# yongjianxu/ompi-release

Hardware: AMD Instinct MI355X
Metric: MPI_Allreduce busbw GB/s (1 GiB fp32, np=8) + op/hip reduce HBM GB/s (higher is better)
Workload: dtype f32; 1 GPU; op/hip 3-buff MPI_SUM MPI_FLOAT, 1 GiB per operand (BASELINE configs[1]); count=268435456, bytes_per_operand=1073741824

## Files before the change

### include/coll_mi355x.h

```cpp
#ifndef MI355X_COLL_MI355X_H
#define MI355X_COLL_MI355X_H

#include "ompi_abi.h"

#ifdef __cplusplus
extern "C" {
#endif

extern mca_coll_base_component_t mca_coll_mi355x_component;

int mca_coll_mi355x_allreduce(void *sbuf, void *rbuf, int count, struct ompi_datatype_t *dtype,
                              struct ompi_op_t *op, struct ompi_communicator_t *comm,
                              mca_coll_base_module_t *module);
int mca_coll_mi355x_reduce(void *sbuf, void *rbuf, int count, struct ompi_datatype_t *dtype, struct ompi_op_t *op,
                           int root, struct ompi_communicator_t *comm, mca_coll_base_module_t *module);
int mca_coll_mi355x_iallreduce(void *sbuf, void *rbuf, int count, struct ompi_datatype_t *dtype, struct ompi_op_t *op,
                               struct ompi_communicator_t *comm, ompi_request_t **request,
                               mca_coll_base_module_t *module);
int mca_coll_mi355x_iscan(void *sbuf, void *rbuf, int count, struct ompi_datatype_t *dtype, struct ompi_op_t *op,
                          struct ompi_communicator_t *comm, ompi_request_t **request, mca_coll_base_module_t *module);
int mca_coll_mi355x_iexscan(void *sbuf, void *rbuf, int count, struct ompi_datatype_t *dtype, struct ompi_op_t *op,
                            struct ompi_communicator_t *comm, ompi_request_t **request, mca_coll_base_module_t *module);
int mca_coll_mi355x_ireduce(void *sbuf, void *rbuf, int count, struct ompi_datatype_t *dtype, struct ompi_op_t *op,
                            int root, struct ompi_communicator_t *comm, ompi_request_t **request,
// ... 72 lines not shown
                                   ompi_request_t **request);
int mca_coll_mi355x_pml_irecv_init(void *buf, size_t count, struct ompi_datatype_t *dt, int src, int tag,
                                   struct ompi_communicator_t *comm, ompi_request_t **request);
int mca_coll_mi355x_pml_start(size_t count, ompi_request_t **requests);

extern int mca_coll_mi355x_priority;
extern int mca_coll_mi355x_allreduce_algorithm;
extern int mca_coll_mi355x_pml_hook;
extern int mca_coll_mi355x_mixed_buffers;
extern int mca_coll_mi355x_rcache_max_maps;
extern unsigned long long mca_coll_mi355x_rcache_size_limit;
extern int mca_coll_mi355x_pipe_min_ranks;
extern int mca_coll_mi355x_pipe_chunk_kib;
extern int mca_coll_mi355x_pipe_wg_per_cu;
extern int mca_coll_mi355x_pipe_wt;
extern unsigned long long mca_coll_mi355x_one_phase_max;
extern unsigned long long mca_coll_mi355x_svc_max;
extern unsigned long long mca_coll_mi355x_svc_pull_max;
extern unsigned long long mca_coll_mi355x_svc_copy_max;
extern int mca_coll_mi355x_svc_idle_us;
extern int mca_coll_mi355x_svc_shrink_us;
extern int mca_coll_mi355x_selftest;
extern int mca_coll_mi355x_nb_order;
extern unsigned long long mca_coll_mi355x_scan_part_min;
struct mi355x_comm *mca_coll_mi355x_engine_of(struct ompi_communicator_t *comm);

extern unsigned long mca_coll_mi355x_staged_calls;
int mca_coll_mi355x_reducible_type(const struct ompi_datatype_t *dt);

#ifdef __cplusplus
// ... 4 lines not shown
```

### include/mi355x_rt.h

```cpp
#ifndef MI355X_RT_H
#define MI355X_RT_H

#include <stddef.h>
#include <stdint.h>

#include "mi355x_types.h"

#ifdef __cplusplus
extern "C" {
#endif

const char *mi355x_last_error(void);
int mi355x_version(void);
int mi355x_device_count(int *count);
int mi355x_set_device(int dev);
int mi355x_get_device(int *dev);
int mi355x_stream_create(void **stream);
int mi355x_stream_destroy(void *stream);
int mi355x_stream_sync(void *stream);
int mi355x_device_sync(void);
int mi355x_malloc(void **p, size_t bytes);
int mi355x_free(void *p);
int mi355x_host_alloc(void **p, size_t bytes);
int mi355x_host_free(void *p);
// ... 23 lines not shown
int mi355x_op_set_threads(int threads);


typedef struct mi355x_comm mi355x_comm_t;

int mi355x_comm_create(const char *key, int rank, int size, int device, mi355x_comm_t **comm);
int mi355x_comm_create_loopback(int size, int device, mi355x_comm_t **comms);
int mi355x_comm_destroy(mi355x_comm_t *comm);
int mi355x_comm_rank(const mi355x_comm_t *comm);
int mi355x_comm_size(const mi355x_comm_t *comm);
int mi355x_comm_barrier(mi355x_comm_t *comm);
int mi355x_comm_vote(mi355x_comm_t *comm, int device, int *engine);
int mi355x_comm_last_algorithm(const mi355x_comm_t *comm);
int mi355x_debug_pipe_token(mi355x_comm_t *comm, int acquire);
int mi355x_debug_token(uint64_t dev_uid, const char *name, int op);

enum mi355x_knob {
    MI355X_KNOB_ALLREDUCE_ALG = 1,
    MI355X_KNOB_REDUCE_ALG = 2,
    MI355X_KNOB_REDUCE_SCATTER_ALG = 3,
    MI355X_KNOB_BLOCKS_PER_CU = 4,
    MI355X_KNOB_TIMEOUT_S = 5,
    MI355X_KNOB_PUSH = 6,
    MI355X_KNOB_IPC_MAX_BYTES = 7,
    MI355X_KNOB_STAGE_BYTES = 8,
    MI355X_KNOB_REDUCE_CHAIN_FANOUT = 10,
    MI355X_KNOB_LL_MAX_BYTES = 9,
    MI355X_KNOB_TIME_PHASES = 11,
    MI355X_KNOB_COPY_BLOCK_KIB = 12,
    MI355X_KNOB_PIPE = 13,
// ... 16 lines not shown
    MI355X_KNOB_FLOWS_FAILED = 30,
    MI355X_KNOB_CREATE_US = 31,
    MI355X_KNOB_SELFTEST_US = 32,
    MI355X_KNOB_SVC_OWNER = 33,
    MI355X_KNOB_SVC_CLAIMS = 34,
    MI355X_KNOB_SVC_IDLE_US = 35,
    MI355X_KNOB_SVC_SHRINK_US = 36,
    MI355X_KNOB_SVC_REGROWS = 37,
    MI355X_KNOB_DEV_SETUP = 38,
    MI355X_KNOB_SETUP_US = 39,
    MI355X_KNOB_SELFTEST = 40,
    MI355X_KNOB_PIPE_CALLS = 41,
    MI355X_KNOB_EXPORT_MISMATCHES = 42,
    MI355X_KNOB_SELFTEST_REUSED = 43,
    MI355X_KNOB_NB_ORDER = 44,
    MI355X_KNOB_SCAN_PART_MIN_BYTES = 45
};
enum mi355x_flow {
    MI355X_FLOW_SVC_LL = 1,
    MI355X_FLOW_SVC_PULL = 2,
    MI355X_FLOW_SVC_COPY = 4,
    MI355X_FLOW_SVC_RS = 8,
    MI355X_FLOW_PIPE = 16
};
int mi355x_comm_set(mi355x_comm_t *comm, int knob, long value);
int mi355x_comm_get(const mi355x_comm_t *comm, int knob, long *value);
int mi355x_comm_phase_ms(const mi355x_comm_t *comm, float *phase1_ms, float *phase2_ms);

enum mi355x_coll_id {
    MI355X_COLL_ALLGATHER = 0, MI355X_COLL_ALLREDUCE = 2, MI355X_COLL_BCAST = 7, MI355X_COLL_REDUCE = 11,
// ... 127 lines not shown
```

### ompi-release_amd/__init__.py

```python
from __future__ import annotations

import ctypes
import os
import pathlib

PKG_DIR = pathlib.Path(__file__).resolve().parent
LIB_DIR = pathlib.Path(os.environ["MI355X_LIB_DIR"]) if os.environ.get("MI355X_LIB_DIR") else PKG_DIR / "lib"
REPO_DIR = PKG_DIR.parent

TYPES = [
    "INT8", "UINT8", "INT16", "UINT16", "INT32", "UINT32", "INT64", "UINT64",
    "F_INTEGER", "F_INTEGER1", "F_INTEGER2", "F_INTEGER4", "F_INTEGER8", "F_INTEGER16",
    "FLOAT", "DOUBLE", "F_REAL", "F_REAL2", "F_REAL4", "F_REAL8", "F_REAL16",
    "F_DOUBLE_PRECISION", "LONG_DOUBLE", "F_LOGICAL", "BOOL",
    "C_FLOAT_COMPLEX", "C_DOUBLE_COMPLEX", "C_LONG_DOUBLE_COMPLEX", "BYTE",
    "F_2REAL", "F_2DOUBLE_PRECISION", "F_2INTEGER",
    "FLOAT_INT", "DOUBLE_INT", "LONG_INT", "2INT", "SHORT_INT", "LONG_DOUBLE_INT", "WCHAR",
]
T = {name: i for i, name in enumerate(TYPES)}
OPS = ["NULL", "MAX", "MIN", "SUM", "PROD", "LAND", "BAND", "LOR", "BOR", "LXOR", "BXOR",
       "MAXLOC", "MINLOC", "REPLACE", "NO_OP"]
OP = {name: i for i, name in enumerate(OPS)}

MI355X_SUCCESS = 0
# ... 73 lines not shown
        "mi355x_op_reduce_3buff": (i, [i, i, vp, vp, vp, sz, vp]),
        "mi355x_op_tune": (i, [i, i, i]),
        "mi355x_op_get_tune": (i, [c.POINTER(i), c.POINTER(i), c.POINTER(i)]),
        "mi355x_op_set_mode": (i, [i]),
        "mi355x_op_get_mode": (i, []),
        "mi355x_op_set_threads": (i, [i]),
        "mi355x_comm_create": (i, [c.c_char_p, i, i, i, c.POINTER(vp)]),
        "mi355x_comm_create_loopback": (i, [i, i, c.POINTER(vp)]),
        "mi355x_comm_destroy": (i, [vp]),
        "mi355x_comm_rank": (i, [vp]),
        "mi355x_comm_size": (i, [vp]),
        "mi355x_comm_barrier": (i, [vp]),
        "mi355x_comm_last_algorithm": (i, [vp]),
        "mi355x_debug_pipe_token": (i, [vp, i]),
        "mi355x_debug_token": (i, [c.c_uint64, c.c_char_p, i]),
        "mi355x_comm_set": (i, [vp, i, c.c_long]),
        "mi355x_comm_phase_ms": (i, [vp, c.POINTER(c.c_float), c.POINTER(c.c_float)]),
        "mi355x_comm_get": (i, [vp, i, c.POINTER(c.c_long)]),
        "mi355x_allreduce": (i, [vp, vp, vp, sz, i, i, vp]),
        "mi355x_reduce_scatter_block": (i, [vp, vp, vp, sz, i, i, vp]),
        "mi355x_reduce": (i, [vp, vp, vp, sz, i, i, i, vp]),
        "mi355x_iallreduce": (i, [vp, vp, vp, sz, i, i, vp, c.POINTER(vp)]),
        "mi355x_ireduce": (i, [vp, vp, vp, sz, i, i, i, vp, c.POINTER(vp)]),
        "mi355x_ireduce_scatter_block": (i, [vp, vp, vp, sz, i, i, vp, c.POINTER(vp)]),
        "mi355x_ireduce_scatter": (i, [vp, vp, vp, c.POINTER(i), i, i, vp, c.POINTER(vp)]),
        "mi355x_iallgather": (i, [vp, vp, vp, sz, vp, c.POINTER(vp)]),
        "mi355x_ibcast": (i, [vp, vp, sz, i, vp, c.POINTER(vp)]),
        "mi355x_request_test": (i, [vp, c.POINTER(i)]),
        "mi355x_request_wait": (i, [vp]),
        "mi355x_request_free": (i, [vp]),
# ... 105 lines not shown


def get_tune() -> tuple[int, int, int]:
    a, b, c = ctypes.c_int(), ctypes.c_int(), ctypes.c_int()
    check(rt().mi355x_op_get_tune(ctypes.byref(a), ctypes.byref(b), ctypes.byref(c)))
    return a.value, b.value, c.value


def scan_part_plan(count: int, n: int, q: int, r: int) -> tuple[int, int, int | None]:
    a, b, c_ = ctypes.c_size_t(), ctypes.c_size_t(), ctypes.c_size_t()
    check(rt().mi355x_scan_part_plan(count, n, q, r, ctypes.byref(a), ctypes.byref(b), ctypes.byref(c_)),
          "mi355x_scan_part_plan")
    return a.value, b.value, None if r == q else c_.value


KNOB = {"ALLREDUCE_ALG": 1, "REDUCE_ALG": 2, "REDUCE_SCATTER_ALG": 3, "BLOCKS_PER_CU": 4, "TIMEOUT_S": 5,
        "PUSH": 6, "IPC_MAX_BYTES": 7, "STAGE_BYTES": 8,
        "LL_MAX_BYTES": 9, "REDUCE_CHAIN_FANOUT": 10, "TIME_PHASES": 11,
        "COPY_BLOCK_KIB": 12, "PIPE": 13, "PIPE_WG_PER_CU": 14, "PIPE_CHUNK_KIB": 15, "PIPE_WT": 16,
        "ONE_PHASE_MAX_BYTES": 17, "PIPE_REFUSED": 18, "SVC_MAX_BYTES": 19, "SVC_CALLS": 20,
        "SVC_LAUNCHES": 21, "SVC_RESIDENT": 22, "SVC_PULL_MAX_BYTES": 23,
        "SVC_PULL_COPY_MAX_BYTES": 24, "RCACHE_MAX_MAPS": 25, "RCACHE_SIZE_LIMIT": 26, "PEER_MAPS": 27,
        "RCACHE_EVICTIONS": 28, "FLOWS": 29, "FLOWS_FAILED": 30, "CREATE_US": 31, "SELFTEST_US": 32,
        "SVC_OWNER": 33, "SVC_CLAIMS": 34, "SVC_IDLE_US": 35,
        "SVC_SHRINK_US": 36, "SVC_REGROWS": 37, "DEV_SETUP": 38, "SETUP_US": 39, "SELFTEST": 40,
        "PIPE_CALLS": 41, "EXPORT_MISMATCHES": 42, "SELFTEST_REUSED": 43, "NB_ORDER": 44,
        "SCAN_PART_MIN_BYTES": 45}
NBC_ALG = {"BINOMIAL": 101, "RING": 102, "CHAIN": 103}
FLOW = {"SVC_LL": 1, "SVC_PULL": 2, "SVC_COPY": 4, "SVC_RS": 8, "PIPE": 16}
COLL = {"ALLGATHER": 0, "ALLREDUCE": 2, "BCAST": 7, "REDUCE": 11, "REDUCESCATTER": 12}
AR_ALG = {"DECISION": 0, "LINEAR": 1, "NONOVERLAPPING": 2, "RECURSIVE_DOUBLING": 3, "RING": 4,
          "RING_SEGMENTED": 5}


class Comm:

    def __init__(self, handle: int):
        self.h = ctypes.c_void_p(handle)

    @classmethod
    def create(cls, key: str, rank: int, size: int, device: int) -> "Comm":
        h = ctypes.c_void_p()
# ... 374 lines not shown
```

### ompi-release_amd/csrc/mca/coll/mi355x/coll_mi355x_component.c

```c
#include <stdio.h>
#include <stdlib.h>
#include <string.h>
#include <time.h>
#include <unistd.h>

#include "../../../../../include/coll_mi355x.h"
#include "../../../../../include/mi355x_rt.h"

int mca_coll_mi355x_priority = 90;
int mca_coll_mi355x_allreduce_algorithm = 0;
int mca_coll_mi355x_pml_hook = 1;

typedef struct mca_coll_mi355x_module_t {
    mca_coll_base_module_t super;
    mi355x_comm_t *engine;
    mca_coll_base_module_allreduce_fn_t prev_allreduce;
    mca_coll_base_module_t *prev_allreduce_module;
    mca_coll_base_module_reduce_scatter_fn_t prev_reduce_scatter;
    mca_coll_base_module_t *prev_reduce_scatter_module;
    mca_coll_base_module_reduce_scatter_block_fn_t prev_reduce_scatter_block;
    mca_coll_base_module_t *prev_reduce_scatter_block_module;
    mca_coll_base_module_allgather_fn_t prev_allgather;
    mca_coll_base_module_t *prev_allgather_module;
    mca_coll_base_module_bcast_fn_t prev_bcast;
// ... 244 lines not shown
    default:
        fprintf(stderr, "[coll/mi355x] %s\n", mi355x_last_error());
        return OMPI_ERROR;
    }
}

#define MOD(m) ((mca_coll_mi355x_module_t *)(m))

int mca_coll_mi355x_mixed_buffers = 1;
int mca_coll_mi355x_rcache_max_maps = 0;
unsigned long long mca_coll_mi355x_rcache_size_limit = 0;
int mca_coll_mi355x_pipe_min_ranks = 4;
int mca_coll_mi355x_pipe_chunk_kib = 0;
int mca_coll_mi355x_pipe_wg_per_cu = 2;
int mca_coll_mi355x_pipe_wt = 1;
unsigned long long mca_coll_mi355x_one_phase_max = 1ull << 20;
unsigned long long mca_coll_mi355x_svc_max = 32ull << 10;
unsigned long long mca_coll_mi355x_svc_pull_max = 128ull << 10;
unsigned long long mca_coll_mi355x_svc_copy_max = 1ull << 20;
int mca_coll_mi355x_svc_idle_us = 1000;
int mca_coll_mi355x_svc_shrink_us = 100;
int mca_coll_mi355x_selftest = 1;
int mca_coll_mi355x_nb_order = 0;
unsigned long long mca_coll_mi355x_scan_part_min = 0;
int mca_coll_mi355x_timeout_s = 0;

static int route(mca_coll_mi355x_module_t *m, int dev)
{
    if (!m->mixed) return dev;
    int engine = dev;
// ... 1740 lines not shown
    return OMPI_ERR_BAD_PARAM;
}

static int apply_engine_params(mca_coll_mi355x_module_t *m, struct ompi_communicator_t *comm)
{
    const int n = mi355x_comm_size_of(comm);
    int rc = OMPI_SUCCESS;
#define KNOB(K, V, NAME) if (rc == OMPI_SUCCESS) rc = set_knob(m, MI355X_KNOB_##K, (long)(V), NAME)
    KNOB(SELFTEST, mca_coll_mi355x_selftest != 0, "selftest");
    KNOB(NB_ORDER, mca_coll_mi355x_nb_order != 0, "nb_order");
    KNOB(SCAN_PART_MIN_BYTES, mca_coll_mi355x_scan_part_min, "scan_part_min_bytes");
    KNOB(PIPE, mca_coll_mi355x_pipe_min_ranks > 0 && n >= mca_coll_mi355x_pipe_min_ranks, "pipe_min_ranks");
    KNOB(PIPE_CHUNK_KIB, mca_coll_mi355x_pipe_chunk_kib, "pipe_chunk_kib");
    KNOB(PIPE_WG_PER_CU, mca_coll_mi355x_pipe_wg_per_cu, "pipe_wg_per_cu");
    KNOB(PIPE_WT, mca_coll_mi355x_pipe_wt != 0, "pipe_wt");
    KNOB(ONE_PHASE_MAX_BYTES, mca_coll_mi355x_one_phase_max, "one_phase_max");
    KNOB(SVC_MAX_BYTES, mca_coll_mi355x_svc_max, "svc_max");
    KNOB(SVC_PULL_MAX_BYTES, mca_coll_mi355x_svc_pull_max, "svc_pull_max");
    KNOB(SVC_PULL_COPY_MAX_BYTES, mca_coll_mi355x_svc_copy_max, "svc_copy_max");
    KNOB(SVC_IDLE_US, mca_coll_mi355x_svc_idle_us, "svc_idle_us");
    KNOB(SVC_SHRINK_US, mca_coll_mi355x_svc_shrink_us, "svc_shrink_us");
    if (mca_coll_mi355x_timeout_s > 0) KNOB(TIMEOUT_S, mca_coll_mi355x_timeout_s, "timeout_s");
#undef KNOB
    return rc;
}

struct mi355x_comm *mca_coll_mi355x_engine_of(struct ompi_communicator_t *comm)
{
    if (!comm || comm->c_coll.coll_allreduce != mca_coll_mi355x_allreduce || !comm->c_coll.coll_allreduce_module)
        return NULL;
// ... 94 lines not shown
                 "allgather / bcast (every rank votes its buffer kind; 0: every rank must use the same kind)",
                 OPAL_INFO_LVL_5, &mca_coll_mi355x_mixed_buffers);
    register_int("rcache_max_maps", "Most mappings of peers' device allocations kept open per communicator; the least "
                 "recently used beyond it are closed (0 = unlimited)", OPAL_INFO_LVL_9, &mca_coll_mi355x_rcache_max_maps);
    register_ull("rcache_size_limit", "The same bound in bytes of mapped peer allocations, as mpool_rgpusm_rcache_size_limit "
                 "(0 = unlimited)", OPAL_INFO_LVL_9, &mca_coll_mi355x_rcache_size_limit);
    register_int("pipe_min_ranks", "Communicators of at least this many ranks run large allreduces through the "
                 "pipelined copy||reduce flow (one persistent launch, per-chunk flags); 0 = never", OPAL_INFO_LVL_5,
                 &mca_coll_mi355x_pipe_min_ranks);
    register_int("pipe_chunk_kib", "Chunk size of the pipelined allreduce in KiB (0 = about 512 chunks per ring block)",
                 OPAL_INFO_LVL_6, &mca_coll_mi355x_pipe_chunk_kib);
    register_int("pipe_wg_per_cu", "Workgroups per CU of the pipelined allreduce (1..8)", OPAL_INFO_LVL_6,
                 &mca_coll_mi355x_pipe_wg_per_cu);
    register_int("pipe_wt", "Pipelined allreduce: 1 = fold results stored write-through with system-scope ready flags, "
                 "0 = stored and released by the producer's fence", OPAL_INFO_LVL_9, &mca_coll_mi355x_pipe_wt);
    register_ull("one_phase_max", "Per-rank message bytes up to which an allreduce runs the one-launch ring-ordered flow "
                 "instead of the two-phase one", OPAL_INFO_LVL_6, &mca_coll_mi355x_one_phase_max);
    register_ull("svc_max", "Per-rank message bytes up to which small allreduce / reduce / allgather / bcast / "
                 "reduce_scatter_block calls go to the resident LL service in its LL form (svc_max, svc_pull_max and "
                 "svc_copy_max all 0: no service)", OPAL_INFO_LVL_5,
                 &mca_coll_mi355x_svc_max);
    register_ull("svc_pull_max", "Per-rank bytes up to which the service serves allreduce in its pull form (above "
                 "svc_max)", OPAL_INFO_LVL_6, &mca_coll_mi355x_svc_pull_max);
    register_ull("svc_copy_max", "Per-rank bytes up to which the service copies allgather / bcast (above svc_max)",
                 OPAL_INFO_LVL_6, &mca_coll_mi355x_svc_copy_max);
    register_int("svc_idle_us", "Idle time after which the resident service's kernel leaves the GPU, microseconds "
                 "(100 .. 60000000)", OPAL_INFO_LVL_6, &mca_coll_mi355x_svc_idle_us);
    register_int("svc_shrink_us", "Idle time after which the resident service shrinks to one workgroup, microseconds "
                 "(0 = never)", OPAL_INFO_LVL_6, &mca_coll_mi355x_svc_shrink_us);
    register_int("selftest", "Run the cross-device flows' self-tests at a communicator's first device-buffer collective "
// ... 85 lines not shown
```

### ompi-release_amd/csrc/rt/coll_comm.cpp

```cpp

#include <fcntl.h>
#include <immintrin.h>
#include <poll.h>
#include <sched.h>
#include <signal.h>
#include <sys/mman.h>
#include <sys/socket.h>
#include <sys/stat.h>
#include <sys/un.h>
#include <unistd.h>

#include <algorithm>
#include <array>
#include <atomic>
#include <cerrno>
#include <chrono>
#include <condition_variable>
#include <cstddef>
#include <deque>
#include <functional>
#include <cstdio>
#include <cstdlib>
#include <cstring>
#include <map>
// ... 349 lines not shown
    case MI355X_KNOB_REDUCE_SCATTER_ALG: *value = c->knob_rs; break;
    case MI355X_KNOB_BLOCKS_PER_CU: *value = c->tune.blocks_per_cu; break;
    case MI355X_KNOB_TIMEOUT_S: *value = (long)c->timeout_s; break;
    case MI355X_KNOB_PUSH: *value = c->tune.push; break;
    case MI355X_KNOB_IPC_MAX_BYTES: *value = (long)c->ipc_max; break;
    case MI355X_KNOB_STAGE_BYTES: *value = (long)c->stage_bytes; break;
    case MI355X_KNOB_PIPE_REFUSED: *value = (long)c->pipe_refused; break;
    case MI355X_KNOB_LL_MAX_BYTES: *value = (long)c->ll_max; break;
    case MI355X_KNOB_REDUCE_CHAIN_FANOUT: *value = c->chain_fanout; break;
    case MI355X_KNOB_TIME_PHASES: *value = c->time_phases ? 1 : 0; break;
    case MI355X_KNOB_COPY_BLOCK_KIB: *value = c->tune.copy_block_kib; break;
    case MI355X_KNOB_PIPE: *value = c->pipe_on ? 1 : 0; break;
    case MI355X_KNOB_PIPE_WG_PER_CU: *value = c->tune.pipe_wg_per_cu; break;
    case MI355X_KNOB_PIPE_CHUNK_KIB: *value = c->tune.pipe_chunk_kib; break;
    case MI355X_KNOB_PIPE_WT: *value = c->tune.pipe_wt; break;
    case MI355X_KNOB_ONE_PHASE_MAX_BYTES: *value = (long)c->one_phase_max; break;
    case MI355X_KNOB_SVC_MAX_BYTES: *value = svc_limit_visible(c) ? (long)c->svc_max : 0; break;
    case MI355X_KNOB_SVC_CALLS: *value = (long)c->svc_calls; break;
    case MI355X_KNOB_SVC_LAUNCHES: *value = (long)c->svc_launches; break;
    case MI355X_KNOB_SVC_RESIDENT: *value = c->svcq && svc_resident(c->svcq) ? 1 : 0; break;
    case MI355X_KNOB_SVC_PULL_MAX_BYTES: *value = svc_limit_visible(c) ? (long)c->svc_pull_max : 0; break;
    case MI355X_KNOB_SVC_PULL_COPY_MAX_BYTES: *value = svc_limit_visible(c) ? (long)c->svc_copy_max : 0; break;
    case MI355X_KNOB_FLOWS: *value = (long)c->flows; break;
    case MI355X_KNOB_FLOWS_FAILED: *value = (long)c->flows_failed; break;
    case MI355X_KNOB_CREATE_US: *value = (long)c->create_us; break;
    case MI355X_KNOB_SELFTEST_US: *value = (long)c->selftest_us; break;
    case MI355X_KNOB_SELFTEST_REUSED: *value = (long)c->selftest_reused; break;
    case MI355X_KNOB_DEV_SETUP: *value = c->dev_ready ? 1 : 0; break;
    case MI355X_KNOB_SELFTEST: *value = c->selftest ? 1 : 0; break;
    case MI355X_KNOB_PIPE_CALLS: *value = (long)c->pipe_calls; break;
// ... 64 lines not shown
        break;
    case MI355X_KNOB_COPY_BLOCK_KIB:
        if (value < 4 || value > 256) return set_error(MI355X_ERR_ARG, "copy_block_kib out of range");
        c->tune.copy_block_kib = (int)value;
        break;
    case MI355X_KNOB_PIPE: c->pipe_on = value != 0 && (c->flows & MI355X_FLOW_PIPE); break;
    case MI355X_KNOB_PIPE_WG_PER_CU:
        if (value < 1 || value > 8) return set_error(MI355X_ERR_ARG, "pipe_wg_per_cu out of range");
        c->tune.pipe_wg_per_cu = (int)value;
        break;
    case MI355X_KNOB_PIPE_CHUNK_KIB:
        if (value < 0 || value > (1l << 20)) return set_error(MI355X_ERR_ARG, "pipe_chunk_kib out of range");
        c->tune.pipe_chunk_kib = (int)value;
        break;
    case MI355X_KNOB_PIPE_WT: c->tune.pipe_wt = value != 0; break;
    case MI355X_KNOB_ONE_PHASE_MAX_BYTES:
        if (value < 0 || value > (1l << 30)) return set_error(MI355X_ERR_ARG, "one_phase_max_bytes out of range");
        c->one_phase_max = (size_t)value;
        break;
    case MI355X_KNOB_TIME_PHASES:
        c->time_phases = value != 0;
        if (c->time_phases && !c->tev[0]) {
            DeviceGuard dg(c->device);
            for (hipEvent_t &e : c->tev) MI_HIP(hipEventCreate(&e));
        }
        break;
    case MI355X_KNOB_LL_MAX_BYTES:
        if (value < 0 || value > (64l << 20)) return set_error(MI355X_ERR_ARG, "ll_max_bytes out of range");
        c->ll_max = c->ll_ok ? (size_t)value : 0;
        break;
// ... 121 lines not shown
```

### ompi-release_amd/csrc/rt/coll_internal.hpp

```cpp
#pragma once

#include <hip/hip_runtime.h>

#include <cstddef>
#include <cstdint>

namespace mi355x {

constexpr int kMaxRanks = 64;
constexpr int kFoldChunk = 8;
constexpr int kTreeMax = 16;
constexpr int kTreeSteps = 64;

struct FoldArgs {
    const void *src[kMaxRanks];
    void *dst[kMaxRanks];
    int order[kMaxRanks];
    uint64_t role_mask;
    int nr;
    int nd;
    size_t n;
    size_t head, nvec;
    int three;
};
// ... 120 lines not shown
    const void *src[kMaxRanks];
    const char *peer_rbuf[kMaxRanks];
    char *dst;
    uint64_t *peer_flag[kMaxRanks];
    const uint64_t *my_flag;
    uint64_t *queue;
    uint32_t *err;
    uint64_t qbase, seq, timeout_ticks, kmax, chunk, count;
    uint64_t boff[kMaxRanks], blen[kMaxRanks];
    uint64_t role_mask;
    uint64_t co_pull;
    int order[kMaxRanks];
    int n, me, co_fold;
    int wt;
    uint32_t nchunks;
    uint64_t *dbg;
};
int launch_pipe_slot(int op, int type, const PipeArgs &a, unsigned grid, hipStream_t s);
int pipe_blocks_per_cu(int op, int type, size_t count);

struct CollTune {
    int blocks_per_cu = 1024;
    int copy_block_kib = 4;
    int push = 0;
    int pipe_wg_per_cu = 2;
    int pipe_chunk_kib = 0;
    int pipe_wt = 1;
};
CollTune &coll_tune();
CollTune &coll_tune_default();
CollTune *coll_tune_use(CollTune *t);

int launch_fold_slot(int op, int type, const FoldArgs &a, hipStream_t s);
int launch_scan_slot(int op, int type, const ScanArgs &a, hipStream_t s);
int launch_ring_all_slot(int op, int type, const RingAllArgs &a, hipStream_t s);
int launch_tree_slot(int op, int type, const TreeArgs &a, hipStream_t s);
int launch_copy(CopyArgs a, hipStream_t s);
int launch_multicopy(MultiCopyArgs a, hipStream_t s);

}
```

### ompi-release_amd/csrc/rt/coll_pipe.hip

```cpp
#include "coll_internal.hpp"
#include "op_functors.hpp"
#include "rt_internal.hpp"
#include "slot_list.hpp"

namespace mi355x {

typedef unsigned int u32x4p __attribute__((ext_vector_type(4)));

template <typename T> struct alignas(16) PVec {
    T e[16 / sizeof(T)];
};

template <bool NT> __device__ __forceinline__ u32x4p pload(const void *p)
{
    if constexpr (NT) return __builtin_nontemporal_load(reinterpret_cast<const u32x4p *>(p));
    return *reinterpret_cast<const u32x4p *>(p);
}
template <bool NT> __device__ __forceinline__ void pstore(void *p, const u32x4p &v)
{
    if constexpr (NT) __builtin_nontemporal_store(v, reinterpret_cast<u32x4p *>(p));
    else *reinterpret_cast<u32x4p *>(p) = v;
}

constexpr int kSysCoherent = 1 | 16;
// ... 142 lines not shown
}

template <class F, bool NT> __global__ __launch_bounds__(256) void k_pipe_allreduce(PipeArgs a)
{
    using T = typename F::T;
    constexpr size_t esz = sizeof(T);
    __shared__ uint64_t item_s;
    __shared__ uint32_t give_up_s;
    const uint64_t total = (uint64_t)a.nchunks * (uint64_t)a.n;
    for (;;) {
        if (threadIdx.x == 0) item_s = __hip_atomic_fetch_add(a.queue, 1ull, __ATOMIC_RELAXED, __HIP_MEMORY_SCOPE_AGENT) - a.qbase;
        __syncthreads();
        const uint64_t it = uniform64(item_s);
        if (threadIdx.x == 0) dbg_store(a, 0, it);
        if (it >= total) break;
        if (it < a.nchunks) {
            const uint64_t k = it;
            const size_t blen = a.blen[a.me], lo = k * a.chunk, hi = lo + a.chunk < blen ? lo + a.chunk : blen;
            const bool wt = a.wt && a.co_fold && ((uintptr_t)(a.dst + (a.boff[a.me] + lo) * esz) & 15) == 0 &&
                            (((hi - lo) * esz) & 15) == 0;
            if (lo < hi) fold_range<F, NT>(a, a.boff[a.me] + lo, a.boff[a.me] + hi, wt);
            asm volatile("s_waitcnt vmcnt(0)" ::: "memory");
            __syncthreads();
            if (threadIdx.x == 0) {
                if (!wt) __builtin_amdgcn_fence(__ATOMIC_RELEASE, "");
                asm volatile("s_waitcnt vmcnt(0)" ::: "memory");
                for (int q = 0; q < a.n; ++q)
                    if (q != a.me) __hip_atomic_store(a.peer_flag[q] + k, a.seq, __ATOMIC_RELAXED, __HIP_MEMORY_SCOPE_SYSTEM);
                dbg_store(a, 1, 2);
            }
        } else {
            const uint64_t j = it - a.nchunks;
            const uint64_t k = j / (uint64_t)(a.n - 1);
            const int q = (int)((a.me + 1 + (int)(j % (uint64_t)(a.n - 1))) % a.n);
            const size_t blen = a.blen[q], lo = k * a.chunk, hi = lo + a.chunk < blen ? lo + a.chunk : blen;
            const size_t b0 = (a.boff[q] + lo) * esz, b1 = (a.boff[q] + hi) * esz;
            const bool co = (a.co_pull >> q) & 1u;
            const bool wt = a.wt && co && ((uintptr_t)(a.dst + b0) & 15) == 0 && ((b1 - b0) & 15) == 0;
            if (threadIdx.x == 0) {
                uint32_t give_up = 0;
                const uint64_t *f = a.my_flag + (size_t)q * a.kmax + k;
                const uint64_t t0 = __builtin_amdgcn_s_memrealtime();
                unsigned polls = 0;
                while (flag_load(f) < a.seq) {
                    __builtin_amdgcn_s_sleep(2);
                    if ((++polls & 1023u) == 0 &&
                        (__hip_atomic_load(a.err, __ATOMIC_RELAXED, __HIP_MEMORY_SCOPE_SYSTEM) != 0 ||
                         __builtin_amdgcn_s_memrealtime() - t0 > a.timeout_ticks)) {
                        __hip_atomic_store(a.err, 1u, __ATOMIC_RELAXED, __HIP_MEMORY_SCOPE_SYSTEM);
// ... 75 lines not shown
```

### ompi-release_amd/csrc/rt/coll_pipe_host.cpp

```cpp

#include <fcntl.h>
#include <immintrin.h>
#include <poll.h>
#include <sched.h>
#include <signal.h>
#include <sys/mman.h>
#include <sys/socket.h>
#include <sys/stat.h>
#include <sys/un.h>
#include <unistd.h>

#include <algorithm>
#include <array>
#include <atomic>
#include <cerrno>
#include <chrono>
#include <condition_variable>
#include <cstddef>
#include <deque>
#include <functional>
#include <cstdio>
#include <cstdlib>
#include <cstring>
#include <map>
// ... 26 lines not shown
    MI_HIP(hipMemsetAsync(c->pipe_queue, 0, sizeof(uint64_t), ss));
    if (!c->ll_err) MI_HIP(hipHostMalloc((void **)&c->ll_err, sizeof(uint32_t), hipHostMallocCoherent));
    MI_HIP(hipStreamSynchronize(ss));
    c->pipe_kmax = kPipeKmax;
    c->pipe_qbase = 0;
    c->pipe_seq = 0;
    const void *mine[1] = {c->pipe_base};
    const uint64_t sig[4] = {11, bytes, 0, 0};
    std::vector<std::vector<void *>> P;
    int rc = exchange(c, 1, mine, sig, P, nullptr, true, true);
    if (rc) return rc;
    c->pipe_peer.assign(n, nullptr);
    for (size_t q = 0; q < n; ++q) c->pipe_peer[q] = (char *)P[0][q];
    TRACE(c, "pipe region %zu bytes, %d ranks on this GPU", bytes, c->pipe_share);
    return barrier(c);
}

}

namespace mi355x {

int pipe_allreduce(mi355x_comm *c, int op, int type, const Program &pr,
                          const std::vector<std::vector<void *>> &P, size_t count, hipStream_t s)
{
    if (!c->pipe_base) return set_error(MI355X_ERR_ARG, "pipelined allreduce before its setup");
    int rc = MI355X_SUCCESS;
    const size_t esz = mi355x_type_size(type), n = (size_t)c->size;
    PipeArgs a;
    std::memset(&a, 0, sizeof(a));
    size_t maxlen = 0;
// ... 35 lines not shown
    for (size_t j = 0; j < pr.order.size(); ++j) a.order[j] = pr.order[j];
    a.role_mask = pr.role_mask;
    const uintptr_t m = (uintptr_t)a.dst & 15;
    a.wt = coll_tune().pipe_wt;
    a.co_fold = (m % esz) == 0;
    for (int q = 0; q < c->size && a.co_fold; ++q) a.co_fold = (((uintptr_t)a.src[q]) & 15) == m;
    for (int q = 0; q < c->size; ++q)
        if ((((uintptr_t)a.peer_rbuf[q]) & 15) == m) a.co_pull |= 1ull << q;
    const uint64_t total = (uint64_t)nchunks * n;
    const int share = std::max(1, c->pipe_share);
    int wpc = coll_tune().pipe_wg_per_cu;
    if (share > 1) wpc = std::min(wpc, pipe_blocks_per_cu(op, type, count));
    uint64_t grid = (uint64_t)std::max(1, wpc * device_cu_count() / share);
    if (share == 1) grid = std::max<uint64_t>(grid, 8);
    if (grid > total) grid = total;
    const bool tp = c->time_phases && c->tev[0];
    if (tp) MI_HIP(hipEventRecord(c->tev[0], s));
    TRACE(c, "pipe launch seq %llu grid %llu chunks %zu x %zu elements qbase %llu co_fold %d co_pull %llx",
          (unsigned long long)a.seq, (unsigned long long)grid, nchunks, chunk, (unsigned long long)a.qbase, a.co_fold,
          (unsigned long long)a.co_pull);
    if (debug_on()) {
        if (!c->pipe_dbg) MI_HIP(hipHostMalloc((void **)&c->pipe_dbg, 4 * 4096 * sizeof(uint64_t), hipHostMallocCoherent));
        std::memset(c->pipe_dbg, 0, 4 * 4096 * sizeof(uint64_t));
        if (grid <= 4096) a.dbg = c->pipe_dbg;
    }
    rc = launch_pipe_slot(op, type, a, (unsigned)grid, s);
    if (rc) return rc;
    if (tp) MI_HIP(hipEventRecord(c->tev[1], s));
    if (a.dbg) {
        const auto t0 = std::chrono::steady_clock::now();
        double next = 2.0;
        while (hipStreamQuery(s) == hipErrorNotReady) {
            usleep(1000);
            const double el = std::chrono::duration<double>(std::chrono::steady_clock::now() - t0).count();
// ... 98 lines not shown
```

### ompi-release_amd/csrc/rt/coll_selftest.cpp

```cpp

#include <fcntl.h>
#include <immintrin.h>
#include <poll.h>
#include <sched.h>
#include <signal.h>
#include <sys/mman.h>
#include <sys/socket.h>
#include <sys/stat.h>
#include <sys/un.h>
#include <unistd.h>

#include <algorithm>
#include <array>
#include <atomic>
#include <cerrno>
#include <chrono>
#include <condition_variable>
#include <cstddef>
#include <deque>
#include <functional>
#include <cstdio>
#include <cstdlib>
#include <cstring>
#include <map>
// ... 215 lines not shown
    const int n = c->size;
    const size_t count = (size_t)n * 32768;
    struct Saved {
        bool pipe, want;
        size_t one;
        int ar;
        const mi355x_rules_t *rules;
        double timeout;
    } sv{c->pipe_on, c->svc_want, c->one_phase_max, c->knob_allreduce, c->rules, c->timeout_s};
    c->pipe_on = true;
    c->svc_want = false;
    c->one_phase_max = 0;
    c->knob_allreduce = AR_RING;
    c->rules = nullptr;
    c->pipe_chunk_override = 4096;
    c->timeout_s = env_double("MI355X_LL_PROBE_S", 5.0);
    unsigned pass = 0;
    bool admitted = false;
    {
        SelfTest st(c, 0x9e37u, count * 4);
        std::vector<uint32_t> h;
        const uint64_t refused = c->pipe_refused;
        bool ok = st.prepare(7, count) &&
                  allreduce_impl(c, st.in, st.out, count, MI355X_T_INT32, MI355X_OP_SUM, st.s) == MI355X_SUCCESS &&
                  st.fetch(h, count);
        for (size_t i = 0; i < count && ok; ++i) ok = h[i] == st.sum(7, i);
        admitted = c->pipe_refused == refused;
        if (ok) pass |= MI355X_FLOW_PIPE;
        (void)hipGetLastError();
    }
    c->pipe_on = sv.pipe;
    c->svc_want = sv.want;
    c->one_phase_max = sv.one;
    c->knob_allreduce = sv.ar;
    c->rules = sv.rules;
    c->timeout_s = sv.timeout;
    c->pipe_chunk_override = 0;
    pass &= ~selftest_injected();
    unsigned all = 0;
    int rc = agree_flows(c, (pass | ~(unsigned)MI355X_FLOW_PIPE) | (admitted ? 0u : (unsigned)MI355X_FLOW_PIPE), &all);
    if (rc) return rc;
    c->pipe_untested = !admitted;
    if (!(all & MI355X_FLOW_PIPE)) {
        c->flows &= ~(unsigned)MI355X_FLOW_PIPE;
        c->flows_failed |= MI355X_FLOW_PIPE;
        c->pipe_on = false;
        if (c->rank == 0)
            fprintf(stderr, "[mi355x] pipelined allreduce self-test failed: large allreduces take the two-phase flow\n");
    }
    c->selftest_us += std::chrono::duration<double, std::micro>(std::chrono::steady_clock::now() - t0).count();
    TRACE(c, "pipelined flow self-test: %s", !admitted ? "not admitted (untested)" : (all & MI355X_FLOW_PIPE) ? "ok" : "failed -> off");
    return MI355X_SUCCESS;
// ... 211 lines not shown
```

### ompi-release_amd/csrc/rt/comm_internal.hpp

```cpp
#pragma once

#include <unistd.h>

#include <atomic>
#include <condition_variable>
#include <cstdint>
#include <cstdio>
#include <cstdlib>
#include <deque>
#include <functional>
#include <map>
#include <memory>
#include <mutex>
#include <string>
#include <thread>
#include <vector>

#include "coll_internal.hpp"
#include "coll_sched.hpp"
#include "rt_internal.hpp"
#include "svc_queue.hpp"

namespace mi355x {

// ... 247 lines not shown
    size_t svc_copy_max = (size_t)1 << 20;
    bool svc_rs = true;
    bool svc_keep = false;
    bool svc_want = false;
    bool svc_attached = false;
    bool svc_flows_tested = false;
    int selftest_reused = 0;
    uint64_t svc_epoch = 0;
    uint64_t svc_tries = 0;
    uint64_t svc_retry = 16;
    uint64_t svc_revocations = 0;
    double svc_handover_s = 0.01;
    unsigned flows = 0x1f, flows_failed = 0;
    bool pipe_untested = false;
    size_t pipe_chunk_override = 0;
    bool gated = false;
    uint64_t gate_calls = 0;
    size_t ll_bytes = 0;
    double create_us = 0, selftest_us = 0;
    void *gf_buf = nullptr;
    size_t gf_bytes = 0;
    double gf_used = 0;
    mi355x::CollTune tune = mi355x::coll_tune_default();
    uint64_t use_clock = 0;
    bool dev_ready = false;
    bool selftest = true;
    double setup_us = 0;
    std::vector<std::pair<int, long>> preset;
    bool svc_stuck = false;
    uint64_t *svc_trace = nullptr;
// ... 86 lines not shown
```

Baseline: 6613 GB/s.

## Interleave pipelined allreduce pulls with folds using a bounded lag in the work queue

```diff
diff --git a/include/coll_mi355x.h b/include/coll_mi355x.h
--- a/include/coll_mi355x.h
+++ b/include/coll_mi355x.h
@@ -110,6 +110,7 @@
 extern int mca_coll_mi355x_pipe_chunk_kib;
 extern int mca_coll_mi355x_pipe_wg_per_cu;
 extern int mca_coll_mi355x_pipe_wt;
+extern int mca_coll_mi355x_pipe_lag;
 extern unsigned long long mca_coll_mi355x_one_phase_max;
 extern unsigned long long mca_coll_mi355x_svc_max;
 extern unsigned long long mca_coll_mi355x_svc_pull_max;
diff --git a/include/mi355x_rt.h b/include/mi355x_rt.h
--- a/include/mi355x_rt.h
+++ b/include/mi355x_rt.h
@@ -61,6 +61,8 @@
 int mi355x_comm_last_algorithm(const mi355x_comm_t *comm);
 int mi355x_debug_pipe_token(mi355x_comm_t *comm, int acquire);
 int mi355x_debug_token(uint64_t dev_uid, const char *name, int op);
+int mi355x_debug_pipe_item(uint32_t item, uint32_t nchunks, int n, int me, long lag, int *kind, uint32_t *chunk, int *peer);
+long mi355x_debug_pipe_lag(long knob, int share, size_t chunk_bytes, uint64_t grid, int n);
 
 enum mi355x_knob {
     MI355X_KNOB_ALLREDUCE_ALG = 1,
@@ -107,6 +109,7 @@
     MI355X_KNOB_EXPORT_MISMATCHES = 42,
     MI355X_KNOB_SELFTEST_REUSED = 43,
     MI355X_KNOB_NB_ORDER = 44,
+    MI355X_KNOB_PIPE_LAG = 46,
     MI355X_KNOB_SCAN_PART_MIN_BYTES = 45
 };
 enum mi355x_flow {
diff --git a/ompi-release_amd/__init__.py b/ompi-release_amd/__init__.py
--- a/ompi-release_amd/__init__.py
+++ b/ompi-release_amd/__init__.py
@@ -111,6 +111,9 @@
         "mi355x_comm_last_algorithm": (i, [vp]),
         "mi355x_debug_pipe_token": (i, [vp, i]),
         "mi355x_debug_token": (i, [c.c_uint64, c.c_char_p, i]),
+        "mi355x_debug_pipe_item": (i, [c.c_uint32, c.c_uint32, i, i, c.c_long, c.POINTER(i), c.POINTER(c.c_uint32),
+                                       c.POINTER(i)]),
+        "mi355x_debug_pipe_lag": (c.c_long, [c.c_long, i, sz, c.c_uint64, i]),
         "mi355x_comm_set": (i, [vp, i, c.c_long]),
         "mi355x_comm_phase_ms": (i, [vp, c.POINTER(c.c_float), c.POINTER(c.c_float)]),
         "mi355x_comm_get": (i, [vp, i, c.POINTER(c.c_long)]),
@@ -246,6 +249,17 @@
     return a.value, b.value, None if r == q else c_.value
 
 
+def pipe_item(item: int, nchunks: int, n: int, me: int, lag: int) -> tuple[int, int, int]:
+    kind, chunk, peer = ctypes.c_int(), ctypes.c_uint32(), ctypes.c_int()
+    check(rt().mi355x_debug_pipe_item(item, nchunks, n, me, lag, ctypes.byref(kind), ctypes.byref(chunk),
+                                      ctypes.byref(peer)), "mi355x_debug_pipe_item")
+    return kind.value, chunk.value, peer.value
+
+
+def pipe_lag(knob: int, share: int, chunk_bytes: int, grid: int, n: int) -> int:
+    return int(rt().mi355x_debug_pipe_lag(knob, share, chunk_bytes, grid, n))
+
+
 KNOB = {"ALLREDUCE_ALG": 1, "REDUCE_ALG": 2, "REDUCE_SCATTER_ALG": 3, "BLOCKS_PER_CU": 4, "TIMEOUT_S": 5,
         "PUSH": 6, "IPC_MAX_BYTES": 7, "STAGE_BYTES": 8,
         "LL_MAX_BYTES": 9, "REDUCE_CHAIN_FANOUT": 10, "TIME_PHASES": 11,
@@ -257,7 +271,7 @@
         "SVC_OWNER": 33, "SVC_CLAIMS": 34, "SVC_IDLE_US": 35,
         "SVC_SHRINK_US": 36, "SVC_REGROWS": 37, "DEV_SETUP": 38, "SETUP_US": 39, "SELFTEST": 40,
         "PIPE_CALLS": 41, "EXPORT_MISMATCHES": 42, "SELFTEST_REUSED": 43, "NB_ORDER": 44,
-        "SCAN_PART_MIN_BYTES": 45}
+        "SCAN_PART_MIN_BYTES": 45, "PIPE_LAG": 46}
 NBC_ALG = {"BINOMIAL": 101, "RING": 102, "CHAIN": 103}
 FLOW = {"SVC_LL": 1, "SVC_PULL": 2, "SVC_COPY": 4, "SVC_RS": 8, "PIPE": 16}
 COLL = {"ALLGATHER": 0, "ALLREDUCE": 2, "BCAST": 7, "REDUCE": 11, "REDUCESCATTER": 12}
diff --git a/ompi-release_amd/csrc/mca/coll/mi355x/coll_mi355x_component.c b/ompi-release_amd/csrc/mca/coll/mi355x/coll_mi355x_component.c
--- a/ompi-release_amd/csrc/mca/coll/mi355x/coll_mi355x_component.c
+++ b/ompi-release_amd/csrc/mca/coll/mi355x/coll_mi355x_component.c
@@ -282,6 +282,7 @@
 int mca_coll_mi355x_pipe_chunk_kib = 0;
 int mca_coll_mi355x_pipe_wg_per_cu = 2;
 int mca_coll_mi355x_pipe_wt = 1;
+int mca_coll_mi355x_pipe_lag = -2;
 unsigned long long mca_coll_mi355x_one_phase_max = 1ull << 20;
 unsigned long long mca_coll_mi355x_svc_max = 32ull << 10;
 unsigned long long mca_coll_mi355x_svc_pull_max = 128ull << 10;
@@ -2052,6 +2053,7 @@
     KNOB(PIPE_CHUNK_KIB, mca_coll_mi355x_pipe_chunk_kib, "pipe_chunk_kib");
     KNOB(PIPE_WG_PER_CU, mca_coll_mi355x_pipe_wg_per_cu, "pipe_wg_per_cu");
     KNOB(PIPE_WT, mca_coll_mi355x_pipe_wt != 0, "pipe_wt");
+    KNOB(PIPE_LAG, mca_coll_mi355x_pipe_lag, "pipe_lag");
     KNOB(ONE_PHASE_MAX_BYTES, mca_coll_mi355x_one_phase_max, "one_phase_max");
     KNOB(SVC_MAX_BYTES, mca_coll_mi355x_svc_max, "svc_max");
     KNOB(SVC_PULL_MAX_BYTES, mca_coll_mi355x_svc_pull_max, "svc_pull_max");
@@ -2176,6 +2178,9 @@
                  &mca_coll_mi355x_pipe_wg_per_cu);
     register_int("pipe_wt", "Pipelined allreduce: 1 = fold results stored write-through with system-scope ready flags, "
                  "0 = stored and released by the producer's fence", OPAL_INFO_LVL_9, &mca_coll_mi355x_pipe_wt);
+    register_int("pipe_lag", "Pipelined allreduce: chunks the pulls stay behind the folds in a rank's work queue "
+                 "(-1 = every fold first, -2 = from the ranks sharing the GPU and the chunk size)", OPAL_INFO_LVL_6,
+                 &mca_coll_mi355x_pipe_lag);
     register_ull("one_phase_max", "Per-rank message bytes up to which an allreduce runs the one-launch ring-ordered flow "
                  "instead of the two-phase one", OPAL_INFO_LVL_6, &mca_coll_mi355x_one_phase_max);
     register_ull("svc_max", "Per-rank message bytes up to which small allreduce / reduce / allgather / bcast / "
diff --git a/ompi-release_amd/csrc/rt/coll_comm.cpp b/ompi-release_amd/csrc/rt/coll_comm.cpp
--- a/ompi-release_amd/csrc/rt/coll_comm.cpp
+++ b/ompi-release_amd/csrc/rt/coll_comm.cpp
@@ -387,6 +387,7 @@
     case MI355X_KNOB_PIPE_WG_PER_CU: *value = c->tune.pipe_wg_per_cu; break;
     case MI355X_KNOB_PIPE_CHUNK_KIB: *value = c->tune.pipe_chunk_kib; break;
     case MI355X_KNOB_PIPE_WT: *value = c->tune.pipe_wt; break;
+    case MI355X_KNOB_PIPE_LAG: *value = c->tune.pipe_lag; break;
     case MI355X_KNOB_ONE_PHASE_MAX_BYTES: *value = (long)c->one_phase_max; break;
     case MI355X_KNOB_SVC_MAX_BYTES: *value = svc_limit_visible(c) ? (long)c->svc_max : 0; break;
     case MI355X_KNOB_SVC_CALLS: *value = (long)c->svc_calls; break;
@@ -481,6 +482,10 @@
         c->tune.pipe_chunk_kib = (int)value;
         break;
     case MI355X_KNOB_PIPE_WT: c->tune.pipe_wt = value != 0; break;
+    case MI355X_KNOB_PIPE_LAG:
+        if (value < -2 || value > 1024) return set_error(MI355X_ERR_ARG, "pipe_lag out of range");
+        c->tune.pipe_lag = (int)value;
+        break;
     case MI355X_KNOB_ONE_PHASE_MAX_BYTES:
         if (value < 0 || value > (1l << 30)) return set_error(MI355X_ERR_ARG, "one_phase_max_bytes out of range");
         c->one_phase_max = (size_t)value;
diff --git a/ompi-release_amd/csrc/rt/coll_internal.hpp b/ompi-release_amd/csrc/rt/coll_internal.hpp
--- a/ompi-release_amd/csrc/rt/coll_internal.hpp
+++ b/ompi-release_amd/csrc/rt/coll_internal.hpp
@@ -158,8 +158,28 @@
     int n, me, co_fold;
     int wt;
     uint32_t nchunks;
+    uint32_t lag;
     uint64_t *dbg;
 };
+struct PipeItem {
+    uint32_t pull;
+    uint32_t chunk;
+    uint32_t j;
+};
+__host__ __device__ inline PipeItem pipe_item(uint32_t it, uint32_t C, uint32_t n, uint32_t L)
+{
+    if (L > C) L = C;
+    if (it < L) return {0u, it, 0u};
+    it -= L;
+    const uint32_t both = (C - L) * n;
+    if (it < both) {
+        const uint32_t g = L + it / n, s = it % n;
+        return s == 0 ? PipeItem{0u, g, 0u} : PipeItem{1u, g - L, s - 1};
+    }
+    it -= both;
+    return {1u, C - L + it / (n - 1), it % (n - 1)};
+}
+long pipe_lag_of(long knob, int share, size_t chunk_bytes, uint64_t grid, int n);
 int launch_pipe_slot(int op, int type, const PipeArgs &a, unsigned grid, hipStream_t s);
 int pipe_blocks_per_cu(int op, int type, size_t count);
 
@@ -170,6 +190,7 @@
     int pipe_wg_per_cu = 2;
     int pipe_chunk_kib = 0;
     int pipe_wt = 1;
+    int pipe_lag = -2;
 };
 CollTune &coll_tune();
 CollTune &coll_tune_default();
diff --git a/ompi-release_amd/csrc/rt/coll_pipe.hip b/ompi-release_amd/csrc/rt/coll_pipe.hip
--- a/ompi-release_amd/csrc/rt/coll_pipe.hip
+++ b/ompi-release_amd/csrc/rt/coll_pipe.hip
@@ -180,8 +180,9 @@
         const uint64_t it = uniform64(item_s);
         if (threadIdx.x == 0) dbg_store(a, 0, it);
         if (it >= total) break;
-        if (it < a.nchunks) {
-            const uint64_t k = it;
+        const PipeItem pi = pipe_item((uint32_t)it, a.nchunks, (uint32_t)a.n, a.lag);
+        if (!pi.pull) {
+            const uint64_t k = pi.chunk;
             const size_t blen = a.blen[a.me], lo = k * a.chunk, hi = lo + a.chunk < blen ? lo + a.chunk : blen;
             const bool wt = a.wt && a.co_fold && ((uintptr_t)(a.dst + (a.boff[a.me] + lo) * esz) & 15) == 0 &&
                             (((hi - lo) * esz) & 15) == 0;
@@ -196,9 +197,8 @@
                 dbg_store(a, 1, 2);
             }
         } else {
-            const uint64_t j = it - a.nchunks;
-            const uint64_t k = j / (uint64_t)(a.n - 1);
-            const int q = (int)((a.me + 1 + (int)(j % (uint64_t)(a.n - 1))) % a.n);
+            const uint64_t k = pi.chunk;
+            const int q = (a.me + 1 + (int)pi.j) % a.n;
             const size_t blen = a.blen[q], lo = k * a.chunk, hi = lo + a.chunk < blen ? lo + a.chunk : blen;
             const size_t b0 = (a.boff[q] + lo) * esz, b1 = (a.boff[q] + hi) * esz;
             const bool co = (a.co_pull >> q) & 1u;
diff --git a/ompi-release_amd/csrc/rt/coll_pipe_host.cpp b/ompi-release_amd/csrc/rt/coll_pipe_host.cpp
--- a/ompi-release_amd/csrc/rt/coll_pipe_host.cpp
+++ b/ompi-release_amd/csrc/rt/coll_pipe_host.cpp
@@ -64,6 +64,37 @@
     for (size_t q = 0; q < n; ++q) c->pipe_peer[q] = (char *)P[0][q];
     TRACE(c, "pipe region %zu bytes, %d ranks on this GPU", bytes, c->pipe_share);
     return barrier(c);
+}
+
+constexpr size_t kPipeLagBytes = (size_t)64 << 20;
+long pipe_lag_of(long knob, int share, size_t chunk_bytes, uint64_t grid, int n)
+{
+    if (knob != -2) return knob;
+    const size_t by_grid = (size_t)((grid + (uint64_t)std::max(1, n) - 1) / (uint64_t)std::max(1, n));
+    const size_t by_bytes = kPipeLagBytes / ((size_t)std::max(1, share) * std::max<size_t>(1, chunk_bytes));
+    return (long)std::min<size_t>(std::max<size_t>(1, std::max(by_grid, by_bytes)), kPipeKmax);
+}
+
+}
+
+extern "C" {
+
+int mi355x_debug_pipe_item(uint32_t item, uint32_t nchunks, int n, int me, long lag, int *kind, uint32_t *chunk, int *peer)
+{
+    using namespace mi355x;
+    if (!kind || !chunk || !peer || n < 2 || n > kMaxRanks || me < 0 || me >= n || nchunks < 1 || nchunks > kPipeKmax ||
+        lag < -1 || item >= nchunks * (uint32_t)n)
+        return set_error(MI355X_ERR_ARG, "bad pipe item arguments");
+    const PipeItem pi = pipe_item(item, nchunks, (uint32_t)n, lag < 0 || lag > (long)nchunks ? nchunks : (uint32_t)lag);
+    *kind = (int)pi.pull;
+    *chunk = pi.chunk;
+    *peer = pi.pull ? (me + 1 + (int)pi.j) % n : me;
+    return MI355X_SUCCESS;
+}
+
+long mi355x_debug_pipe_lag(long knob, int share, size_t chunk_bytes, uint64_t grid, int n)
+{
+    return mi355x::pipe_lag_of(knob, share, chunk_bytes, grid, n);
 }
 
 }
@@ -129,10 +160,13 @@
     uint64_t grid = (uint64_t)std::max(1, wpc * device_cu_count() / share);
     if (share == 1) grid = std::max<uint64_t>(grid, 8);
     if (grid > total) grid = total;
+    const long lag = pipe_lag_of(c->pipe_lag_override != -2 ? c->pipe_lag_override : coll_tune().pipe_lag, share,
+                                 chunk * esz, grid, c->size);
+    a.lag = lag < 0 || (size_t)lag > nchunks ? (uint32_t)nchunks : (uint32_t)lag;
     const bool tp = c->time_phases && c->tev[0];
     if (tp) MI_HIP(hipEventRecord(c->tev[0], s));
-    TRACE(c, "pipe launch seq %llu grid %llu chunks %zu x %zu elements qbase %llu co_fold %d co_pull %llx",
-          (unsigned long long)a.seq, (unsigned long long)grid, nchunks, chunk, (unsigned long long)a.qbase, a.co_fold,
+    TRACE(c, "pipe launch seq %llu grid %llu chunks %zu x %zu elements lag %u qbase %llu co_fold %d co_pull %llx",
+          (unsigned long long)a.seq, (unsigned long long)grid, nchunks, chunk, a.lag, (unsigned long long)a.qbase, a.co_fold,
           (unsigned long long)a.co_pull);
     if (debug_on()) {
         if (!c->pipe_dbg) MI_HIP(hipHostMalloc((void **)&c->pipe_dbg, 4 * 4096 * sizeof(uint64_t), hipHostMallocCoherent));
diff --git a/ompi-release_amd/csrc/rt/coll_selftest.cpp b/ompi-release_amd/csrc/rt/coll_selftest.cpp
--- a/ompi-release_amd/csrc/rt/coll_selftest.cpp
+++ b/ompi-release_amd/csrc/rt/coll_selftest.cpp
@@ -253,6 +253,7 @@
     c->knob_allreduce = AR_RING;
     c->rules = nullptr;
     c->pipe_chunk_override = 4096;
+    c->pipe_lag_override = 2;
     c->timeout_s = env_double("MI355X_LL_PROBE_S", 5.0);
     unsigned pass = 0;
     bool admitted = false;
@@ -275,6 +276,7 @@
     c->rules = sv.rules;
     c->timeout_s = sv.timeout;
     c->pipe_chunk_override = 0;
+    c->pipe_lag_override = -2;
     pass &= ~selftest_injected();
     unsigned all = 0;
     int rc = agree_flows(c, (pass | ~(unsigned)MI355X_FLOW_PIPE) | (admitted ? 0u : (unsigned)MI355X_FLOW_PIPE), &all);
diff --git a/ompi-release_amd/csrc/rt/comm_internal.hpp b/ompi-release_amd/csrc/rt/comm_internal.hpp
--- a/ompi-release_amd/csrc/rt/comm_internal.hpp
+++ b/ompi-release_amd/csrc/rt/comm_internal.hpp
@@ -285,6 +285,7 @@
     unsigned flows = 0x1f, flows_failed = 0;
     bool pipe_untested = false;
     size_t pipe_chunk_override = 0;
+    int pipe_lag_override = -2;
     bool gated = false;
     uint64_t gate_calls = 0;
     size_t ll_bytes = 0;
```

Result: no change. 6613 GB/s (-0.0%).
